# LewisClifton/Deep-Super-Resolution

Hardware: AMD Instinct MI355X
Metric: HR Mpixels/sec x4 GAN train step; PSNR delta vs reference (higher is better)
Workload: dtype bf16; 1 GPU; gan_x4: full GAN step x4 (G + D + VGG19 perceptual), batch 32/GPU, 128x128->512x512; global_batch=32, parallelism=dp1

## Files before the change

### deep-super-resolution_amd/csrc/conv_wgrad_tile.hip

```cpp
#include "dsr_common.h"
#include "dsr_kernels.h"

__device__ __forceinline__ s16x4 tr_read(const unsigned char* p) {
  return __builtin_amdgcn_ds_read_tr16_b64_v4i16((__attribute__((address_space(3))) s16x4*)(p));
}
__device__ __forceinline__ U4 tr_frag(const unsigned char* base, int p1, int p2, int chunk, int within) {
  s16x4 lo = tr_read(base + p1 * 128 + ((chunk ^ (p1 & 7)) << 4) + within);
  s16x4 hi = tr_read(base + p2 * 128 + ((chunk ^ (p2 & 7)) << 4) + within);
  return __builtin_bit_cast(U4, __builtin_shufflevector(lo, hi, 0, 1, 2, 3, 4, 5, 6, 7));
}

template <int DT, int KH, int KW, int S>
__global__ __launch_bounds__(256, 2) void conv_wgrad_tile_kernel(const WgradTileArgs a) {
  constexpr int R = (S == 1) ? 4 : 2;
  constexpr int HR = (R - 1) * S + KH, HC = 31 * S + KW;
  constexpr int NT = KH * KW;
  __shared__ __attribute__((aligned(16))) unsigned char sX[HR * HC * 128];
  __shared__ __attribute__((aligned(16))) unsigned char sY[R * 32 * 128];

  const int tid = threadIdx.x, lane = tid & 63, wave = __builtin_amdgcn_readfirstlane(tid >> 6);
  const int wr = wave >> 1, wc = wave & 1;
  const int g = lane >> 4, l16 = lane & 15, q4 = l16 >> 2, cc = 4 * (l16 & 3);
  const int pair = blockIdx.x;
  const int co0 = (pair / a.tiles_ci) * 64, ci0 = (pair % a.tiles_ci) * 64;
  const unsigned short* __restrict__ X = reinterpret_cast<const unsigned short*>(a.x);
  const unsigned short* __restrict__ DY = reinterpret_cast<const unsigned short*>(a.dy);

  f32x4 acc[NT][2][2];
#pragma unroll
  for (int t = 0; t < NT; ++t)
#pragma unroll
    for (int i = 0; i < 2; ++i)
#pragma unroll
      for (int j = 0; j < 2; ++j) acc[t][i][j] = f32x4{0.f, 0.f, 0.f, 0.f};

  const int c = tid & 7, pbase = tid >> 3;
  const bool yc_ok = (co0 + c * 8) < a.CoutP, xc_ok = (ci0 + c * 8) < a.CinP;
  int t_end = (blockIdx.y + 1) * a.tiles_per_block;
  if (t_end > a.ntiles) t_end = a.ntiles;
  const int per_img = a.tiles_y * a.tiles_x;

  for (int t = blockIdx.y * a.tiles_per_block; t < t_end; ++t) {
    const int n = t / per_img;
    const int rem = t - n * per_img;
    const int oy0 = (rem / a.tiles_x) * R, ox0 = (rem % a.tiles_x) * 32;
    __syncthreads();
#pragma unroll
    for (int i = 0; i < R * 32 * 8 / 256; ++i) {
      const int p = pbase + 32 * i;
      const int oy = oy0 + (p >> 5), ox = ox0 + (p & 31);
      const bool ok = yc_ok && oy < a.OH && ox < a.OW;
      U4 v = load16_or_zero(DY, ((size_t)(n * a.OH + oy) * a.OW + ox) * a.CoutP + co0 + c * 8, ok);
      *reinterpret_cast<U4*>(sY + p * 128 + ((c ^ (p & 7)) << 4)) = v;
    }
    {
      constexpr int NV = (HR * HC + 31) / 32;
      U4 v[NV];
#pragma unroll
      for (int u = 0; u < NV; ++u) {
        const int q = pbase + 32 * u;
        const int hr = q / HC, hc = q - hr * HC;
        bool ok = xc_ok && q < HR * HC;
        const int iy = pad_index(oy0 * S + hr - a.pad, a.IH, a.pad_mode, ok);
        const int ix = pad_index(ox0 * S + hc - a.pad, a.IW, a.pad_mode, ok);
        v[u] = load16_or_zero(X, ((size_t)(n * a.IH + iy) * a.IW + ix) * a.CinP + ci0 + c * 8, ok);
      }
#pragma unroll
      for (int u = 0; u < NV; ++u) {
        const int q = pbase + 32 * u;
        if (q < HR * HC) *reinterpret_cast<U4*>(sX + q * 128 + ((c ^ (q & 7)) << 4)) = v[u];
      }
    }
    __syncthreads();
#pragma unroll 1
    for (int r = 0; r < R; ++r) {
      U4 fa[2];
#pragma unroll
      for (int i = 0; i < 2; ++i) {
        const int ch = wr * 32 + i * 16 + cc;
        fa[i] = tr_frag(sY, r * 32 + 4 * g + q4, r * 32 + 16 + 4 * g + q4, ch >> 3, (ch & 7) * 2);
      }
#pragma unroll
      for (int kh = 0; kh < KH; ++kh)
#pragma unroll
        for (int kw = 0; kw < KW; ++kw) {
          const int qb = (r * S + kh) * HC + kw;
          const int q1 = qb + (4 * g + q4) * S, q2 = qb + (16 + 4 * g + q4) * S;
          U4 fb[2];
#pragma unroll
          for (int j = 0; j < 2; ++j) {
            const int ch = wc * 32 + j * 16 + cc;
            fb[j] = tr_frag(sX, q1, q2, ch >> 3, (ch & 7) * 2);
          }
#pragma unroll
          for (int i = 0; i < 2; ++i)
#pragma unroll
            for (int j = 0; j < 2; ++j) acc[kh * KW + kw][i][j] = mfma16<DT>(fa[i], fb[j], acc[kh * KW + kw][i][j]);
        }
    }
  }

  float* P = a.partial + (size_t)blockIdx.y * NT * a.CoutP * a.CinP;
#pragma unroll
  for (int t = 0; t < NT; ++t)
#pragma unroll
    for (int i = 0; i < 2; ++i)
#pragma unroll
      for (int j = 0; j < 2; ++j)
#pragma unroll
        for (int r = 0; r < 4; ++r) {
          const int co = co0 + wr * 32 + i * 16 + 4 * g + r, ci = ci0 + wc * 32 + j * 16 + l16;
          if (co < a.CoutP && ci < a.CinP) P[((size_t)t * a.CoutP + co) * a.CinP + ci] = acc[t][i][j][r];
        }
}

template <int DT>
__device__ __forceinline__ void conv_wgrad_dma_body(const WgradTileArgs& a, const int pair, const int ychunk) {
  constexpr int R = 2, HC = 40, HR = R + 2;
  constexpr int XB = HR * HC * 128, YB = R * 32 * 128, STAGE = XB + YB;
  __shared__ __attribute__((aligned(16))) unsigned char smem[2 * STAGE];

  const int tid = threadIdx.x, lane = tid & 63, wave = __builtin_amdgcn_readfirstlane(tid >> 6);
  const int g = lane >> 4, l16 = lane & 15, q4 = l16 >> 2, cc = 4 * (l16 & 3);
  const int co0 = (pair / a.tiles_ci) * 64, ci0 = (pair % a.tiles_ci) * 64;

  f32x4 acc[9][4];
#pragma unroll
  for (int t = 0; t < 9; ++t)
#pragma unroll
    for (int i = 0; i < 4; ++i) acc[t][i] = f32x4{0.f, 0.f, 0.f, 0.f};

  const int lp = 4 * g + q4;
  int offA[4], offB[3];
#pragma unroll
  for (int i = 0; i < 4; ++i) {
    const int ch = i * 16 + cc;
    offA[i] = XB + lp * 128 + (((ch >> 3) ^ (lp & 7)) << 4) + (ch & 7) * 2;
  }
#pragma unroll
  for (int kw = 0; kw < 3; ++kw) {
    const int ch = wave * 16 + cc;
    offB[kw] = lp * 128 + (((ch >> 3) ^ ((kw + lp) & 7)) << 4) + (ch & 7) * 2;
  }

  const int chunk = (tid & 7) ^ ((tid >> 3) & 7), pb = tid >> 3;
  const bool yc_ok = (co0 + chunk * 8) < a.CoutP, xc_ok = (ci0 + chunk * 8) < a.CinP;
  const BufSrd xrsrc = make_srd(const_cast<void*>(a.x), a.x_bytes);
  const BufSrd yrsrc = make_srd(const_cast<void*>(a.dy), a.dy_bytes);
  constexpr unsigned OOB = 0xFFFFFFF0u;
  typedef __attribute__((address_space(3))) void* lds_ptr;
  const int per_img = a.tiles_y * a.tiles_x;
  constexpr int NX = (HR * HC) / 32, NY = (R * 32) / 32;
  constexpr int FAR = 0x7FFFFF00;
  int xpart[NX], ypart[NY];
  unsigned hc_pack = 0;
#pragma unroll
  for (int u = 0; u < NX; ++u) {
    const int q = pb + 32 * u;
    const int hr = q / HC, hc = q - hr * HC;
    xpart[u] = (xc_ok && hc < 34) ? ((hr * a.IW + hc) * a.CinP + ci0 + chunk * 8) * 2 : FAR;
    hc_pack |= (unsigned)hc << (6 * u);
  }
#pragma unroll
  for (int u = 0; u < NY; ++u) {
    const int p = pb + 32 * u;
    ypart[u] = yc_ok ? (((p >> 5) * a.OW + (p & 31)) * a.CoutP + co0 + chunk * 8) * 2 : FAR;
  }
  const unsigned ximg = (unsigned)(a.IH * a.IW * a.CinP * 2), yimg = (unsigned)(a.OH * a.OW * a.CoutP * 2);
  const bool fast = a.pad_mode == DSR_PAD_ZERO;
  struct TileXY {
    int n, ty, tx;
  };
  auto dma = [&](const TileXY& tc, int buf) {
    const int n = tc.n;
    const int oy0 = tc.ty * R, ox0 = tc.tx * 32;
    unsigned char* st = smem + buf * STAGE;
    if (fast) {
      const BufSrd xr = make_srd(const_cast<unsigned char*>(reinterpret_cast<const unsigned char*>(a.x)) + (size_t)n * ximg, ximg);
      const BufSrd yr = make_srd(const_cast<unsigned char*>(reinterpret_cast<const unsigned char*>(a.dy)) + (size_t)n * yimg, yimg);
      const int xs = ((oy0 - a.pad) * a.IW + ox0 - a.pad) * a.CinP * 2;
      const int ys = (oy0 * a.OW + ox0) * a.CoutP * 2;
      unsigned char* dx = st + 8 * wave * 128;
      if (ox0 - a.pad >= 0 && ox0 - a.pad + 34 <= a.IW) {
#pragma unroll
        for (int u = 0; u < NX; ++u)
          lds_dma16(xr, dx + 32 * u * 128, (unsigned)(xpart[u] + xs));
      } else {
#pragma unroll
        for (int u = 0; u < NX; ++u) {
          const int ix = ox0 - a.pad + (int)((hc_pack >> (6 * u)) & 63);
          lds_dma16(xr, dx + 32 * u * 128, (unsigned)ix < (unsigned)a.IW ? (unsigned)(xpart[u] + xs) : OOB);
        }
      }
      if (ox0 + 32 <= a.OW) {
#pragma unroll
        for (int u = 0; u < NY; ++u)
          lds_dma16(yr, dx + XB + 32 * u * 128, (unsigned)(ypart[u] + ys));
      } else {
#pragma unroll
        for (int u = 0; u < NY; ++u)
          lds_dma16(yr, dx + XB + 32 * u * 128, ox0 + (pb & 31) < a.OW ? (unsigned)(ypart[u] + ys) : OOB);
      }
      return;
    }
#pragma unroll
    for (int u = 0; u < (HR * HC) / 32; ++u) {
      const int q = pb + 32 * u;
      const int hr = q / HC, hc = q - hr * HC;
      bool ok = xc_ok && hc < 34;
      const int iy = pad_index(oy0 + hr - a.pad, a.IH, a.pad_mode, ok);
      const int ix = pad_index(ox0 + hc - a.pad, a.IW, a.pad_mode, ok);
      lds_dma16(xrsrc, st + (32 * u + 8 * wave) * 128, ok ? (unsigned)((((n * a.IH + iy) * a.IW + ix) * a.CinP + ci0 + chunk * 8) * 2) : OOB);
    }
#pragma unroll
    for (int u = 0; u < (R * 32) / 32; ++u) {
      const int p = pb + 32 * u;
      const int oy = oy0 + (p >> 5), ox = ox0 + (p & 31);
      const bool ok = yc_ok && oy < a.OH && ox < a.OW;
      lds_dma16(yrsrc, st + XB + (32 * u + 8 * wave) * 128, ok ? (unsigned)((((n * a.OH + oy) * a.OW + ox) * a.CoutP + co0 + chunk * 8) * 2) : OOB);
    }
  };
  auto next_tile = [&](TileXY c) {
    if (++c.tx == a.tiles_x) {
      c.tx = 0;
      if (++c.ty == a.tiles_y) {
        c.ty = 0;
        ++c.n;
      }
    }
    return c;
  };

  int t = ychunk * a.tiles_per_block;
  int t_end = t + a.tiles_per_block;
  if (t_end > a.ntiles) t_end = a.ntiles;
  TileXY nxt;
  nxt.n = t / per_img;
  nxt.ty = (t - nxt.n * per_img) / a.tiles_x;
  nxt.tx = t - nxt.n * per_img - nxt.ty * a.tiles_x;
  __builtin_amdgcn_s_setprio(1);
  if (t < t_end) dma(nxt, 0);
  int buf = 0;
  for (; t < t_end; ++t, buf ^= 1) {
    asm volatile("s_waitcnt vmcnt(0)" ::: "memory");
    __builtin_amdgcn_s_barrier();
    asm volatile("" ::: "memory");
    nxt = next_tile(nxt);
    if (t + 1 < t_end) dma(nxt, buf ^ 1);
    __builtin_amdgcn_s_setprio(0);
    const unsigned char* st = smem + buf * STAGE;
    auto frag = [&](int off) {
      const s16x4 lo = tr_read(st + off);
      const s16x4 hi = tr_read(st + off + 2048);
      return __builtin_bit_cast(U4, __builtin_shufflevector(lo, hi, 0, 1, 2, 3, 4, 5, 6, 7));
    };
    constexpr int NU = 3 * HR;
    auto load_b = [&](int u) {
      const int kw = u / HR, h = u - kw * HR;
      return frag(offB[kw] + (h * HC + kw) * 128);
    };
    U4 fa[R][4], fb[3];
#pragma unroll
    for (int i = 0; i < 4; ++i) fa[0][i] = frag(offA[i]);
    fb[0] = load_b(0);
    fb[1] = load_b(1);
#pragma unroll
    for (int r = 1; r < R; ++r)
#pragma unroll
      for (int i = 0; i < 4; ++i) fa[r][i] = frag(offA[i] + r * 32 * 128);
#pragma unroll
    for (int u = 0; u < NU; ++u) {
      if (u + 2 < NU) fb[(u + 2) % 3] = load_b(u + 2);
      __builtin_amdgcn_sched_barrier(0);
      const int kw = u / HR, h = u - kw * HR;
#pragma unroll
      for (int r = 0; r < R; ++r) {
        const int kh = h - r;
        if (kh < 0 || kh > 2) continue;
#pragma unroll
        for (int i = 0; i < 4; ++i) acc[kh * 3 + kw][i] = mfma16<DT>(fa[r][i], fb[u % 3], acc[kh * 3 + kw][i]);
      }
      __builtin_amdgcn_sched_barrier(0);
    }
    __builtin_amdgcn_s_setprio(1);
  }

  float* P = a.partial + (size_t)ychunk * 9 * a.CoutP * a.CinP;
#pragma unroll
  for (int tp = 0; tp < 9; ++tp)
#pragma unroll
    for (int i = 0; i < 4; ++i)
#pragma unroll
      for (int r = 0; r < 4; ++r) {
        const int co = co0 + i * 16 + 4 * g + r, ci = ci0 + wave * 16 + l16;
        if (co < a.CoutP && ci < a.CinP) P[((size_t)tp * a.CoutP + co) * a.CinP + ci] = acc[tp][i][r];
      }
}

template <int DT>
__global__ __launch_bounds__(256, 2) void conv_wgrad_dma_kernel(const WgradTileArgs a) {
  conv_wgrad_dma_body<DT>(a, blockIdx.x, blockIdx.y);
}

template <int DT>
__global__ __launch_bounds__(256, 2) void conv_wgrad_dma_batch_kernel(const WgradBatchArgs b) {
  int pi = 0;
  while (pi + 1 < b.count && (int)blockIdx.x >= b.first_block[pi + 1]) ++pi;
  pi = __builtin_amdgcn_readfirstlane(pi);
  const WgradTileArgs a = b.p[pi];
  const int local = (int)blockIdx.x - b.first_block[pi];
  const int pairs = a.tiles_co * a.tiles_ci;
  conv_wgrad_dma_body<DT>(a, local % pairs, local / pairs);
}

template <int DT, int COH = 1>
__global__ __launch_bounds__(256 * COH, 2) void conv_wgrad_dma_s2_kernel(const WgradTileArgs a) {
  constexpr int HC = 80, HR = 3, NSLOT = HR * HC;
  constexpr int XB = NSLOT * 128, YB = 32 * 128, STAGE = XB + COH * YB;
  __shared__ __attribute__((aligned(16))) unsigned char smem[2 * STAGE];

  const int tid = threadIdx.x & 255, lane = tid & 63, wave = __builtin_amdgcn_readfirstlane((threadIdx.x >> 6) & 3);
  const int hsel = __builtin_amdgcn_readfirstlane(threadIdx.x >> 8);
  const int g = lane >> 4, l16 = lane & 15, q4 = l16 >> 2, cc = 4 * (l16 & 3);
  const int pair = blockIdx.x;
  const int co0 = (pair / a.tiles_ci) * 64 * COH + hsel * 64, ci0 = (pair % a.tiles_ci) * 64;

  f32x4 acc[9][4];
#pragma unroll
  for (int t = 0; t < 9; ++t)
#pragma unroll
    for (int i = 0; i < 4; ++i) acc[t][i] = f32x4{0.f, 0.f, 0.f, 0.f};

  const int lp = 4 * g + q4;
  int offA[4], offB[2];
#pragma unroll
  for (int i = 0; i < 4; ++i) {
    const int ch = i * 16 + cc;
    offA[i] = XB + hsel * YB + lp * 128 + (((ch >> 3) ^ (lp & 7)) << 4) + (ch & 7) * 2;
  }
#pragma unroll
  for (int v = 0; v < 2; ++v) {
    const int ch = wave * 16 + cc;
    offB[v] = 2 * lp * 128 + (((ch >> 3) ^ ((lp + v) & 7)) << 4) + (ch & 7) * 2;
  }

  const int pb = tid >> 3;
  const int xchunk = (tid & 7) ^ ((4 * wave + (lane >> 4)) & 7);
  const int ychunk = (tid & 7) ^ ((tid >> 3) & 7);
  const bool yc_ok = (co0 + ychunk * 8) < a.CoutP, xc_ok = (ci0 + xchunk * 8) < a.CinP;
  const BufSrd xrsrc = make_srd(const_cast<void*>(a.x), a.x_bytes);
  const BufSrd yrsrc = make_srd(const_cast<void*>(a.dy), a.dy_bytes);
  constexpr unsigned OOB = 0xFFFFFFF0u;
  typedef __attribute__((address_space(3))) void* lds_ptr;
  const int per_img = a.tiles_y * a.tiles_x;
  constexpr int NX = (NSLOT + 31) / 32;
  constexpr int FAR = 0x7FFFFF00;
  int xpart[NX];
  unsigned hc_lo = 0, hc_hi = 0;
#pragma unroll
  for (int u = 0; u < NX; ++u) {
    const int q = pb + 32 * u;
    const int hr = q / HC, hc = q - hr * HC;
    xpart[u] = (xc_ok && hc < 65 && hr < HR) ? ((hr * a.IW + hc) * a.CinP + ci0 + xchunk * 8) * 2 : FAR;
    if (u < 4) hc_lo |= (unsigned)hc << (7 * u);
    else hc_hi |= (unsigned)hc << (7 * (u - 4));
  }
  const int ypart = yc_ok ? (pb * a.CoutP + co0 + ychunk * 8) * 2 : FAR;
  const unsigned ximg = (unsigned)(a.IH * a.IW * a.CinP * 2), yimg = (unsigned)(a.OH * a.OW * a.CoutP * 2);
  const bool fast = a.pad_mode == DSR_PAD_ZERO;
  struct TileXY {
    int n, ty, tx;
  };
  auto dma = [&](const TileXY& tc, int buf) {
    const int n = tc.n, oy0 = tc.ty, ox0 = tc.tx * 32;
    unsigned char* st = smem + buf * STAGE;
    if (fast) {
      const BufSrd xr = make_srd(const_cast<unsigned char*>(reinterpret_cast<const unsigned char*>(a.x)) + (size_t)n * ximg, ximg);
      const BufSrd yr = make_srd(const_cast<unsigned char*>(reinterpret_cast<const unsigned char*>(a.dy)) + (size_t)n * yimg, yimg);
      const int ix0 = ox0 * 2 - a.pad;
      const int xs = ((oy0 * 2 - a.pad) * a.IW + ix0) * a.CinP * 2;
      const int ys = (oy0 * a.OW + ox0) * a.CoutP * 2;
      unsigned char* dx = st + 8 * wave * 128;
      const bool interior = ix0 >= 0 && ix0 + 65 <= a.IW;
#pragma unroll
      for (int u = 0; u < NX; ++u) {
        if (COH == 2 && (u & 1) != hsel) continue;
        if (32 * u + 8 * wave < NSLOT) {
          unsigned off = (unsigned)(xpart[u] + xs);
          if (!interior) {
            const int hc = (int)(((u < 4 ? hc_lo >> (7 * u) : hc_hi >> (7 * (u - 4)))) & 127);
            if (!((unsigned)(ix0 + hc) < (unsigned)a.IW)) off = OOB;
          }
          lds_dma16(xr, dx + 32 * u * 128, off);
        }
      }
      lds_dma16(yr, dx + XB + hsel * YB, (ox0 + 32 <= a.OW || ox0 + pb < a.OW) ? (unsigned)(ypart + ys) : OOB);
      return;
    }
#pragma unroll
    for (int u = 0; u < (NSLOT + 31) / 32; ++u) {
      if (COH == 2 && (u & 1) != hsel) continue;
      if (32 * u + 8 * wave < NSLOT) {
        const int q = pb + 32 * u;
        const int hr = q / HC, hc = q - hr * HC;
        bool ok = xc_ok && hc < 65;
        const int iy = pad_index(oy0 * 2 + hr - a.pad, a.IH, a.pad_mode, ok);
        const int ix = pad_index(ox0 * 2 + hc - a.pad, a.IW, a.pad_mode, ok);
        lds_dma16(xrsrc, st + (32 * u + 8 * wave) * 128, ok ? (unsigned)((((n * a.IH + iy) * a.IW + ix) * a.CinP + ci0 + xchunk * 8) * 2) : OOB);
      }
    }
    {
      const int ox = ox0 + pb;
      const bool ok = yc_ok && ox < a.OW;
      lds_dma16(yrsrc, st + XB + hsel * YB + 8 * wave * 128, ok ? (unsigned)((((n * a.OH + oy0) * a.OW + ox) * a.CoutP + co0 + ychunk * 8) * 2) : OOB);
    }
  };

  int t = blockIdx.y * a.tiles_per_block;
  int t_end = t + a.tiles_per_block;
  if (t_end > a.ntiles) t_end = a.ntiles;
  TileXY nxt;
  nxt.n = t / per_img;
  nxt.ty = (t - nxt.n * per_img) / a.tiles_x;
  nxt.tx = t - nxt.n * per_img - nxt.ty * a.tiles_x;
  __builtin_amdgcn_s_setprio(1);
  if (t < t_end) dma(nxt, 0);
  int buf = 0;
  for (; t < t_end; ++t, buf ^= 1) {
    asm volatile("s_waitcnt vmcnt(0)" ::: "memory");
    __builtin_amdgcn_s_barrier();
    asm volatile("" ::: "memory");
    if (++nxt.tx == a.tiles_x) {
      nxt.tx = 0;
      if (++nxt.ty == a.tiles_y) {
        nxt.ty = 0;
        ++nxt.n;
      }
    }
    if (t + 1 < t_end) dma(nxt, buf ^ 1);
    __builtin_amdgcn_s_setprio(0);
    const unsigned char* st = smem + buf * STAGE;
    U4 fa[4], fb[3];
    auto load_b = [&](int u) {
      const int kh = u / 3, kw = u % 3;
      const s16x4 lo = tr_read(st + offB[kw >> 1] + (kh * HC + kw) * 128);
      const s16x4 hi = tr_read(st + offB[kw >> 1] + (kh * HC + kw) * 128 + 32 * 128);
      return __builtin_bit_cast(U4, __builtin_shufflevector(lo, hi, 0, 1, 2, 3, 4, 5, 6, 7));
    };
#pragma unroll
    for (int i = 0; i < 4; ++i) {
      const s16x4 lo = tr_read(st + offA[i]);
      const s16x4 hi = tr_read(st + offA[i] + 2048);
      fa[i] = __builtin_bit_cast(U4, __builtin_shufflevector(lo, hi, 0, 1, 2, 3, 4, 5, 6, 7));
    }
    fb[0] = load_b(0);
    fb[1] = load_b(1);
#pragma unroll
    for (int u = 0; u < 9; ++u) {
      if (u + 2 < 9) fb[(u + 2) % 3] = load_b(u + 2);
      __builtin_amdgcn_sched_barrier(0);
#pragma unroll
      for (int i = 0; i < 4; ++i) acc[u][i] = mfma16<DT>(fa[i], fb[u % 3], acc[u][i]);
      __builtin_amdgcn_sched_barrier(0);
    }
    __builtin_amdgcn_s_setprio(1);
  }

  float* P = a.partial + (size_t)blockIdx.y * 9 * a.CoutP * a.CinP;
#pragma unroll
  for (int tp = 0; tp < 9; ++tp)
#pragma unroll
    for (int i = 0; i < 4; ++i)
#pragma unroll
      for (int r = 0; r < 4; ++r) {
        const int co = co0 + i * 16 + 4 * g + r, ci = ci0 + wave * 16 + l16;
        if (co < a.CoutP && ci < a.CinP) P[((size_t)tp * a.CoutP + co) * a.CinP + ci] = acc[tp][i][r];
      }
}

static bool dsr_wgrad_s2_co128(int KH, int stride, int CoutP, long long x_bytes) {
  const char* e = getenv("DSR_WGRAD_S2_CO128");
  const int mode = e ? atoi(e) : 1;
  if (mode == 0 || KH != 3 || stride != 2 || CoutP < 128 || CoutP % 128 != 0) return false;
  return mode == 2 || x_bytes >= 400ll * 1000 * 1000;
}

int dsr_wgrad_tile_plan(int KH, int KW, int stride, int N, int OH, int OW, int CinP, int CoutP, WgradTileArgs* a) {
  const bool k3 = KH == 3 && KW == 3 && (stride == 1 || stride == 2);
  const bool k1 = KH == 1 && KW == 1 && stride == 1;
  if (!k3 && !k1) return 0;
  const int R = k1 ? 4 : (stride == 1 ? 2 : 1);
  a->tiles_y = (OH + R - 1) / R;
  a->tiles_x = (OW + 31) / 32;
  a->ntiles = N * a->tiles_y * a->tiles_x;
  const bool co128 = dsr_wgrad_s2_co128(KH, stride, CoutP, (long long)N * (2 * OH) * (2 * OW) * CinP * 2);
  a->tiles_co = co128 ? CoutP / 128 : (CoutP + 63) / 64;
  a->tiles_ci = (CinP + 63) / 64;
  long long pairs = (long long)a->tiles_co * a->tiles_ci;
  long long want = ((co128 ? 256 : 512) + pairs - 1) / pairs;
  if (want > a->ntiles) want = a->ntiles;
  if (want < 1) want = 1;
  a->tiles_per_block = (int)((a->ntiles + want - 1) / want);
  return (a->ntiles + a->tiles_per_block - 1) / a->tiles_per_block;
}

template <int DT>
static void launch_dt(const WgradTileArgs& a, int KH, int stride, dim3 grid, hipStream_t st) {
  if (KH == 3 && stride == 1)
    hipLaunchKernelGGL((conv_wgrad_dma_kernel<DT>), grid, dim3(256), 0, st, a);
  else if (KH == 3 && a.tiles_co * 128 == a.CoutP && a.tiles_co * 64 != a.CoutP)
    hipLaunchKernelGGL((conv_wgrad_dma_s2_kernel<DT, 2>), grid, dim3(512), 0, st, a);
  else if (KH == 3)
    hipLaunchKernelGGL((conv_wgrad_dma_s2_kernel<DT>), grid, dim3(256), 0, st, a);
  else
    hipLaunchKernelGGL((conv_wgrad_tile_kernel<DT, 1, 1, 1>), grid, dim3(256), 0, st, a);
}

void dsr_launch_wgrad_dma_batch(const WgradBatchArgs& b, int dtype, hipStream_t st) {
  const int blocks = b.first_block[b.count];
  if (dtype == DSR_DTYPE_BF16)
    hipLaunchKernelGGL((conv_wgrad_dma_batch_kernel<DSR_DTYPE_BF16>), dim3(blocks), dim3(256), 0, st, b);
  else
    hipLaunchKernelGGL((conv_wgrad_dma_batch_kernel<DSR_DTYPE_F16>), dim3(blocks), dim3(256), 0, st, b);
}

void dsr_launch_wgrad_tile(const WgradTileArgs& a, int KH, int stride, int ychunks, int dtype, hipStream_t st) {
  dim3 grid(a.tiles_co * a.tiles_ci, ychunks);
  if (dtype == DSR_DTYPE_BF16)
    launch_dt<DSR_DTYPE_BF16>(a, KH, stride, grid, st);
  else
    launch_dt<DSR_DTYPE_F16>(a, KH, stride, grid, st);
}
```

### deep-super-resolution_amd/csrc/dsr_kernels.h

```cpp
#pragma once
#include <hip/hip_runtime.h>
#include <stdint.h>
#include <stdlib.h>

#define DSR_MAX_TAPS 96
#define DSR_WGRAD_SCRATCH_SLABS 16

#define DSR_F_BIAS 1
#define DSR_F_STATS 2
#define DSR_F_PIXSHUF 4
#define DSR_F_OUT_NCHW_F32 8
#define DSR_F_PRELU_PTR 16
#define DSR_F_AFFINE 32
#define DSR_F_RESIDUAL 64
#define DSR_F_MASK 128

struct FastDiv {
  unsigned magic;
  unsigned shift;
};
static inline FastDiv fd_make(unsigned d) {
  FastDiv f;
  unsigned s = 0;
  while ((1ull << s) < d) ++s;
  f.shift = s;
  f.magic = (unsigned)((((1ull << 32) * ((1ull << s) - d)) / d) + 1);
  return f;
}
#if defined(__HIPCC__)
__device__ __forceinline__ int fd_div(const FastDiv f, int m) {
  return (int)((__umulhi((unsigned)m, f.magic) + (unsigned)m) >> f.shift);
}
#endif

struct ConvGemmArgs {
  const void* x;
  const void* w;
  void* y;
  float* out_f32;
  const float* bias;
  const float* prelu;
  float* stats;
  unsigned x_bytes, w_bytes;
  unsigned y_bytes;
  int M, GH, GW;
  int IH, IW, CinP;
  int OH, OW, CoutP;
  int NB;
  int cout;
  int stats_stride;
  int isy, isx, osy, osx, ooy, oox;
  int ntaps, CU, U, ksteps;
  int pad_mode, act;
  float slope;
  int flags;
  int tiles_m, tiles_n;
  FastDiv fd_ghw, fd_gw, fd_cu, fd_cu8;
  const void* mask_x;
  int mask_act;
  float mask_slope;
  int taps[DSR_MAX_TAPS];
};

void dsr_launch_conv_gemm(const ConvGemmArgs& a, int dtype, hipStream_t st);
static inline int dsr_conv_big_mode(void) {
  const char* e = getenv("DSR_CONV_BIG");
  return e ? atoi(e) : 2;
}
static inline bool dsr_conv_gemm_use_256(long long M, int NB, bool fast, bool stats) {
  const long long tiles = ((M + 255) / 256) * ((NB + 255) / 256);
  (void)stats;
  const char* t = getenv("DSR_CONV_BIG_TILES");
  return dsr_conv_big_mode() == 2 && fast && NB % 256 == 0 && tiles >= (t ? atoi(t) : 150);
}

static inline bool dsr_conv_gemm_use_224(long long M, int NB, bool fast, int flags) {
  const char* e = getenv("DSR_CONV_BM224");
  const int mode = e ? atoi(e) : 1;
  if (mode == 0 || (flags & (DSR_F_STATS | DSR_F_PIXSHUF | DSR_F_OUT_NCHW_F32))) return false;
  if (!dsr_conv_gemm_use_256(M, NB, fast, false)) return false;
  if (mode == 2) return true;
  const long long cus = 256, nt = NB / 256;
  const long long r256 = (((M + 255) / 256) * nt + cus - 1) / cus, r224 = (((M + 223) / 224) * nt + cus - 1) / cus;
  return r224 * 7 < r256 * 8;
}

static inline bool dsr_conv_gemm_use_64(long long M, int NB, bool fast, int flags) {
  const char* e = getenv("DSR_CONV_BM64");
  const int mode = e ? atoi(e) : 1;
  if (mode == 0 || !fast || NB % 128 != 0 || (flags & (DSR_F_STATS | DSR_F_PIXSHUF | DSR_F_OUT_NCHW_F32))) return false;
  if (mode == 2) return true;
  return ((M + 127) / 128) * (NB / 128) < 256;
}

bool dsr_launch_conv_gemm_persist(const ConvGemmArgs& a, int dtype, hipStream_t st);

struct WgradArgs {
  const void* x;
  const void* dy;
  float* partial;
  int M, OH, OW, IH, IW, CinP, CoutP;
  int stride, pad, pad_mode, KH, KW;
  int tiles_co, tiles_ci, splits, chunk;
  FastDiv fd_ohw, fd_ow;
};
void dsr_launch_wgrad(const WgradArgs& a, int dtype, hipStream_t st);

struct WgradTileArgs {
  const void* x;
  const void* dy;
  float* partial;
  int N, OH, OW, IH, IW, CinP, CoutP;
  int pad, pad_mode;
  int tiles_co, tiles_ci;
  int tiles_y, tiles_x, ntiles, tiles_per_block;
  unsigned x_bytes, dy_bytes;
};
#define DSR_WGRAD_BATCH_MAX 36
struct WgradBatchArgs {
  WgradTileArgs p[DSR_WGRAD_BATCH_MAX];
  int first_block[DSR_WGRAD_BATCH_MAX + 1];
  int count;
};
static_assert(sizeof(WgradBatchArgs) <= 4096, "kernel arguments are limited to 4 KB");
void dsr_launch_wgrad_dma_batch(const WgradBatchArgs& b, int dtype, hipStream_t st);
struct WgradReduceBatchArgs {
  struct Entry {
    const float* partial;
    float* dw;
    int splits, Cout, Cin, CoutP, CinP, first_block;
  } e[DSR_WGRAD_BATCH_MAX];
  int count, total_blocks;
};
void dsr_launch_wgrad_reduce_batch(const WgradReduceBatchArgs& r, hipStream_t st);
int dsr_wgrad_tile_plan(int KH, int KW, int stride, int N, int OH, int OW, int CinP, int CoutP, WgradTileArgs* a);
void dsr_launch_wgrad_tile(const WgradTileArgs& a, int KH, int stride, int ychunks, int dtype, hipStream_t st);

int dsr_wgrad_toeplitz_plan(int N, int H, int W, WgradTileArgs* a);
void dsr_launch_wgrad_toeplitz(const WgradTileArgs& a, int dtype, hipStream_t st);
void dsr_launch_dgrad_toeplitz(const void* dy, const void* w_dgrad, void* dx, int N, int H, int W, int dtype, hipStream_t st,
                               const void* act_out = nullptr, const float* prelu = nullptr, void* dyu = nullptr,
                               float* ps_partial = nullptr);
int dsr_dgrad_toeplitz_ps_blocks(int N, int H, int W);
int dsr_wgrad_taps_plan(int KH, int KW, int stride, int N, int OH, int OW, int CinP, int CoutP, WgradTileArgs* a);
void dsr_launch_wgrad_taps(const WgradTileArgs& a, int KH, int ychunks, int dtype, hipStream_t st);

struct SmallNArgs {
  const void* x;
  const void* w;
  void* y;
  float* out_f32;
  const float* bias;
  const float* prelu;
  int IH, IW, CinP, OH, OW, CoutP, NB, cout, KH, KW, pad, act;
  float slope;
  int tiles_y, tiles_x, ntiles;
  int flip;
  unsigned x_bytes;
};
int dsr_launch_conv_smalln(SmallNArgs& a, int N, int dtype, hipStream_t st);

struct C64Args {
  const void* x;
  const void* w;
  void* y;
  const float* bias;
  const float* prelu;
  float* stats;
  const float* scale;
  const float* shift;
  const void* res;
  int H, W;
  int CoutP;
  int act;
  float slope;
  int flags;
  int mask_act;
  float mask_slope;
  int tiles_y, tiles_x, ntiles;
  int tap_y[9], tap_x[9];
  unsigned x_bytes, y_bytes;
};
int dsr_c64_tiles(int N, int H, int W, int tile_rows);
int dsr_c64_stat_rows(int N, int H, int W, int CoutP);
void dsr_launch_conv_c64(C64Args& a, int N, int dtype, hipStream_t st);

struct Cin8Args {
  const void* x;
  const void* w;
  void* y;
  const float* bias;
  const float* prelu;
  int H, W;
  int act;
  float slope;
  int tiles_y, tiles_x, ntiles;
  unsigned x_bytes;
  int nt_store;
};
void dsr_launch_conv_cin8(Cin8Args& a, int N, int dtype, hipStream_t st);
int dsr_conv_rgb9_supported(int KH, int KW, int stride, int pad, int pad_mode, int Cin, int Cout);
void dsr_launch_conv_rgb9(Cin8Args& a, int N, int dtype, hipStream_t st);
struct Rgb9WgradArgs {
  const void* x;
  const void* dy;
  float* partial;
  int H, W;
  int tiles_y, tiles_x, ntiles;
  unsigned x_bytes, dy_bytes;
};
int dsr_wgrad_rgb9_blocks(int N, int H, int W);
size_t dsr_wgrad_rgb9_slab_floats();
void dsr_launch_wgrad_rgb9(Rgb9WgradArgs& a, int N, int Cin, float* dw, int dtype, hipStream_t st);

struct DgradS2Args {
  const void* dy;
  const void* w;
  void* dx;
  int H, W, CinP, CoutP;
  int OH, OW, M, ci_blocks, kblocks, tiles_m;
  unsigned dy_bytes, w_bytes, dx_bytes;
  FastDiv fd_ghw, fd_gw;
  const void* img;
  const float* w0;
  const float* b0;
  float* fb_partial;
  unsigned img_bytes;
  int Cin0, act0;
  float slope0;
  const void* bn_y;
  const float* bn_scale;
  const float* bn_shift;
  float* bn_partial;
  int bn_act;
  float bn_slope;
};
int dsr_dgrad_s2_blocks(int N, int H, int W, int CinP);
bool dsr_dgrad_s2_bn_supported(int KH, int KW, int stride, int pad, int pad_mode, int H, int W, int CinP, int CoutP, int N);
bool dsr_dgrad_s2_supported(int KH, int KW, int stride, int pad, int pad_mode, int H, int W, int CinP, int CoutP, int N);
void dsr_launch_dgrad_s2(DgradS2Args& a, int N, int dtype, hipStream_t st);

struct Halo64Args {
  const void* x;
  const void* w;
  void* y;
  const float* bias;
  int H, W, CinP;
  int mirror;
  int act;
  float slope;
  int flags;
  const void* mask_x;
  int mask_act;
  float mask_slope;
  int cout_full;
  int kblocks, tiles_y, tiles_x, ntiles;
  unsigned w_bytes, y_bytes;
};
bool dsr_halo64_supported(int KH, int KW, int stride, int pad, int pad_mode, int H, int W, int CinP, int CoutP);
void dsr_launch_conv_halo64(Halo64Args& a, int N, int dtype, hipStream_t st);

struct First2Args {
  const void* x;
  const void* w0;
  const float* b0;
  float slope0;
  const void* w1;
  const float* b1;
  void* a0;
  void* y1;
  float* stats;
  int H, W, OH, OW, tiles_y, tiles_x, ntiles;
  unsigned a0_bytes, y1_bytes;
};

struct FirstBwdArgs {
  const void* x;
  const void* dout;
  const void* y;
  float* partial;
  int N, H, W, act;
  float slope;
  int tiles_y, tiles_x, ntiles;
  unsigned x_bytes, y_bytes;
  const float* w0;
  const float* b0;
  int Cin;
};

void dsr_launch_wgrad_reduce(const float* partial, float* dw, int splits, int ntaps, int Cout, int Cin, int CoutP,
                             int CinP, hipStream_t st);

#include <atomic>
struct LdsOptIn {
  std::atomic<unsigned long long> done{0};
  void ensure(const void* fn, int bytes) {
    int dev = 0;
    (void)hipGetDevice(&dev);
    const unsigned long long bit = 1ull << (dev & 63);
    if (!(done.load(std::memory_order_acquire) & bit)) {
      (void)hipFuncSetAttribute(fn, hipFuncAttributeMaxDynamicSharedMemorySize, bytes);
      done.fetch_or(bit, std::memory_order_release);
    }
  }
};

int dsr_launch_status(const char* what);
int dsr_fail(int code, const char* fmt, ...);

#define DSR_REQUIRE(cond, ...)                          \
  do {                                                  \
    if (!(cond)) return dsr_fail(DSR_E_ARG, __VA_ARGS__); \
  } while (0)
#define DSR_DTYPE_OK(dt) ((dt) == DSR_DTYPE_BF16 || (dt) == DSR_DTYPE_F16)
#define DSR_CP_OK(Cp) ((Cp) >= 8 && (Cp) % 8 == 0 && (Cp) <= 2048)
```

Baseline: 247.3 HR Mpixels/s.

## Process two output rows per stride-2 wgrad tile to reuse shared input halo

The stride-2 3x3 weight-gradient kernel now tiles two output rows at a time. The 5-row input halo is loaded once and shared between both rows instead of loading 3 rows per output row, which cuts global-to-LDS traffic. The block index is remapped so consecutive tiles stay on the same XCD, and co128 is forced on in two-row mode. The non-co128 two-row variant splits its rows across two 256-thread halves that write separate partial slabs, which doubles the partial buffer and the reduction work. It also raises register pressure from the larger fa array.

```diff
diff --git a/deep-super-resolution_amd/csrc/conv_wgrad_tile.hip b/deep-super-resolution_amd/csrc/conv_wgrad_tile.hip
--- a/deep-super-resolution_amd/csrc/conv_wgrad_tile.hip
+++ b/deep-super-resolution_amd/csrc/conv_wgrad_tile.hip
@@ -313,17 +313,29 @@
   conv_wgrad_dma_body<DT>(a, local % pairs, local / pairs);
 }
 
-template <int DT, int COH = 1>
-__global__ __launch_bounds__(256 * COH, 2) void conv_wgrad_dma_s2_kernel(const WgradTileArgs a) {
-  constexpr int HC = 80, HR = 3, NSLOT = HR * HC;
-  constexpr int XB = NSLOT * 128, YB = 32 * 128, STAGE = XB + COH * YB;
+template <int DT, int COH, int R>
+__global__ __launch_bounds__((COH == 2 || R == 2) ? 512 : 256, 2) void conv_wgrad_dma_s2_kernel(const WgradTileArgs a) {
+  constexpr int HALVES = (COH == 2 || R == 2) ? 2 : 1;
+  constexpr int RW = COH == 2 ? R : 1;
+  constexpr int HC = 80, HR = 2 * R + 1, NSLOT = HR * HC;
+  constexpr int YB = 32 * 128;
+  constexpr int XB = NSLOT * 128, STAGE = XB + COH * R * YB;
   __shared__ __attribute__((aligned(16))) unsigned char smem[2 * STAGE];
 
   const int tid = threadIdx.x & 255, lane = tid & 63, wave = __builtin_amdgcn_readfirstlane((threadIdx.x >> 6) & 3);
   const int hsel = __builtin_amdgcn_readfirstlane(threadIdx.x >> 8);
+  const int coh = COH == 2 ? hsel : 0;
+  const int row0 = COH == 2 ? 0 : hsel;
   const int g = lane >> 4, l16 = lane & 15, q4 = l16 >> 2, cc = 4 * (l16 & 3);
-  const int pair = blockIdx.x;
-  const int co0 = (pair / a.tiles_ci) * 64 * COH + hsel * 64, ci0 = (pair % a.tiles_ci) * 64;
+  int pair, chunk;
+  {
+    const int total = gridDim.x * gridDim.y, hw = blockIdx.x + blockIdx.y * gridDim.x;
+    const int q = total >> 3, rem = total & 7, xcd = hw & 7, slot = hw >> 3;
+    const int lin = xcd < rem ? xcd * (q + 1) + slot : rem * (q + 1) + (xcd - rem) * q + slot;
+    pair = __builtin_amdgcn_readfirstlane(lin % (int)gridDim.x);
+    chunk = __builtin_amdgcn_readfirstlane(lin / (int)gridDim.x);
+  }
+  const int co0 = (pair / a.tiles_ci) * 64 * COH + coh * 64, ci0 = (pair % a.tiles_ci) * 64;
 
   f32x4 acc[9][4];
 #pragma unroll
@@ -336,12 +348,12 @@
 #pragma unroll
   for (int i = 0; i < 4; ++i) {
     const int ch = i * 16 + cc;
-    offA[i] = XB + hsel * YB + lp * 128 + (((ch >> 3) ^ (lp & 7)) << 4) + (ch & 7) * 2;
+    offA[i] = XB + (coh * R + row0) * YB + lp * 128 + (((ch >> 3) ^ (lp & 7)) << 4) + (ch & 7) * 2;
   }
 #pragma unroll
   for (int v = 0; v < 2; ++v) {
     const int ch = wave * 16 + cc;
-    offB[v] = 2 * lp * 128 + (((ch >> 3) ^ ((lp + v) & 7)) << 4) + (ch & 7) * 2;
+    offB[v] = (2 * row0 * HC + 2 * lp) * 128 + (((ch >> 3) ^ ((lp + v) & 7)) << 4) + (ch & 7) * 2;
   }
 
   const int pb = tid >> 3;
@@ -351,28 +363,32 @@
   const BufSrd xrsrc = make_srd(const_cast<void*>(a.x), a.x_bytes);
   const BufSrd yrsrc = make_srd(const_cast<void*>(a.dy), a.dy_bytes);
   constexpr unsigned OOB = 0xFFFFFFF0u;
-  typedef __attribute__((address_space(3))) void* lds_ptr;
   const int per_img = a.tiles_y * a.tiles_x;
   constexpr int NX = (NSLOT + 31) / 32;
+  constexpr int NXL = HALVES == 2 ? (NX + 1) / 2 : NX;
+  static_assert(NXL <= 8, "halo column packing holds 8 passes");
   constexpr int FAR = 0x7FFFFF00;
-  int xpart[NX];
+  int xpart[NXL];
   unsigned hc_lo = 0, hc_hi = 0;
 #pragma unroll
-  for (int u = 0; u < NX; ++u) {
+  for (int k = 0; k < NXL; ++k) {
+    const int u = HALVES == 2 ? 2 * k + hsel : k;
     const int q = pb + 32 * u;
     const int hr = q / HC, hc = q - hr * HC;
-    xpart[u] = (xc_ok && hc < 65 && hr < HR) ? ((hr * a.IW + hc) * a.CinP + ci0 + xchunk * 8) * 2 : FAR;
-    if (u < 4) hc_lo |= (unsigned)hc << (7 * u);
-    else hc_hi |= (unsigned)hc << (7 * (u - 4));
+    xpart[k] = (xc_ok && hc < 65 && hr < HR) ? ((hr * a.IW + hc) * a.CinP + ci0 + xchunk * 8) * 2 : FAR;
+    if (k < 4) hc_lo |= (unsigned)hc << (7 * k);
+    else hc_hi |= (unsigned)hc << (7 * (k - 4));
   }
   const int ypart = yc_ok ? (pb * a.CoutP + co0 + ychunk * 8) * 2 : FAR;
   const unsigned ximg = (unsigned)(a.IH * a.IW * a.CinP * 2), yimg = (unsigned)(a.OH * a.OW * a.CoutP * 2);
+  const int yrow = a.OW * a.CoutP * 2;
   const bool fast = a.pad_mode == DSR_PAD_ZERO;
   struct TileXY {
     int n, ty, tx;
   };
+  auto fetches_row = [&](int r) { return COH == 2 || R == 1 || r == hsel; };
   auto dma = [&](const TileXY& tc, int buf) {
-    const int n = tc.n, oy0 = tc.ty, ox0 = tc.tx * 32;
+    const int n = tc.n, oy0 = tc.ty * R, ox0 = tc.tx * 32;
     unsigned char* st = smem + buf * STAGE;
     if (fast) {
       const BufSrd xr = make_srd(const_cast<unsigned char*>(reinterpret_cast<const unsigned char*>(a.x)) + (size_t)n * ximg, ximg);
@@ -383,23 +399,26 @@
       unsigned char* dx = st + 8 * wave * 128;
       const bool interior = ix0 >= 0 && ix0 + 65 <= a.IW;
 #pragma unroll
-      for (int u = 0; u < NX; ++u) {
-        if (COH == 2 && (u & 1) != hsel) continue;
+      for (int k = 0; k < NXL; ++k) {
+        const int u = HALVES == 2 ? 2 * k + hsel : k;
         if (32 * u + 8 * wave < NSLOT) {
-          unsigned off = (unsigned)(xpart[u] + xs);
+          unsigned off = (unsigned)(xpart[k] + xs);
           if (!interior) {
-            const int hc = (int)(((u < 4 ? hc_lo >> (7 * u) : hc_hi >> (7 * (u - 4)))) & 127);
+            const int hc = (int)(((k < 4 ? hc_lo >> (7 * k) : hc_hi >> (7 * (k - 4)))) & 127);
             if (!((unsigned)(ix0 + hc) < (unsigned)a.IW)) off = OOB;
           }
           lds_dma16(xr, dx + 32 * u * 128, off);
         }
       }
-      lds_dma16(yr, dx + XB + hsel * YB, (ox0 + 32 <= a.OW || ox0 + pb < a.OW) ? (unsigned)(ypart + ys) : OOB);
+      const bool col_ok = ox0 + 32 <= a.OW || ox0 + pb < a.OW;
+#pragma unroll
+      for (int r = 0; r < R; ++r)
+        if (fetches_row(r)) lds_dma16(yr, dx + XB + (coh * R + r) * YB, col_ok ? (unsigned)(ypart + ys + r * yrow) : OOB);
       return;
     }
 #pragma unroll
-    for (int u = 0; u < (NSLOT + 31) / 32; ++u) {
-      if (COH == 2 && (u & 1) != hsel) continue;
+    for (int k = 0; k < NXL; ++k) {
+      const int u = HALVES == 2 ? 2 * k + hsel : k;
       if (32 * u + 8 * wave < NSLOT) {
         const int q = pb + 32 * u;
         const int hr = q / HC, hc = q - hr * HC;
@@ -409,14 +428,17 @@
         lds_dma16(xrsrc, st + (32 * u + 8 * wave) * 128, ok ? (unsigned)((((n * a.IH + iy) * a.IW + ix) * a.CinP + ci0 + xchunk * 8) * 2) : OOB);
       }
     }
-    {
-      const int ox = ox0 + pb;
-      const bool ok = yc_ok && ox < a.OW;
-      lds_dma16(yrsrc, st + XB + hsel * YB + 8 * wave * 128, ok ? (unsigned)((((n * a.OH + oy0) * a.OW + ox) * a.CoutP + co0 + ychunk * 8) * 2) : OOB);
-    }
+#pragma unroll
+    for (int r = 0; r < R; ++r)
+      if (fetches_row(r)) {
+        const int oy = oy0 + r, ox = ox0 + pb;
+        const bool ok = yc_ok && oy < a.OH && ox < a.OW;
+        lds_dma16(yrsrc, st + XB + (coh * R + r) * YB + 8 * wave * 128,
+                  ok ? (unsigned)((((n * a.OH + oy) * a.OW + ox) * a.CoutP + co0 + ychunk * 8) * 2) : OOB);
+      }
   };
 
-  int t = blockIdx.y * a.tiles_per_block;
+  int t = chunk * a.tiles_per_block;
   int t_end = t + a.tiles_per_block;
   if (t_end > a.ntiles) t_end = a.ntiles;
   TileXY nxt;
@@ -440,33 +462,43 @@
     if (t + 1 < t_end) dma(nxt, buf ^ 1);
     __builtin_amdgcn_s_setprio(0);
     const unsigned char* st = smem + buf * STAGE;
-    U4 fa[4], fb[3];
+    constexpr int HRW = 2 * RW + 1, NU = 3 * HRW;
+    U4 fa[RW][4], fb[3];
     auto load_b = [&](int u) {
-      const int kh = u / 3, kw = u % 3;
-      const s16x4 lo = tr_read(st + offB[kw >> 1] + (kh * HC + kw) * 128);
-      const s16x4 hi = tr_read(st + offB[kw >> 1] + (kh * HC + kw) * 128 + 32 * 128);
+      const int kw = u / HRW, h = u - kw * HRW;
+      const s16x4 lo = tr_read(st + offB[kw >> 1] + (h * HC + kw) * 128);
+      const s16x4 hi = tr_read(st + offB[kw >> 1] + (h * HC + kw) * 128 + 32 * 128);
       return __builtin_bit_cast(U4, __builtin_shufflevector(lo, hi, 0, 1, 2, 3, 4, 5, 6, 7));
     };
 #pragma unroll
-    for (int i = 0; i < 4; ++i) {
-      const s16x4 lo = tr_read(st + offA[i]);
-      const s16x4 hi = tr_read(st + offA[i] + 2048);
-      fa[i] = __builtin_bit_cast(U4, __builtin_shufflevector(lo, hi, 0, 1, 2, 3, 4, 5, 6, 7));
-    }
+    for (int r = 0; r < RW; ++r)
+#pragma unroll
+      for (int i = 0; i < 4; ++i) {
+        const s16x4 lo = tr_read(st + offA[i] + r * YB);
+        const s16x4 hi = tr_read(st + offA[i] + r * YB + 2048);
+        fa[r][i] = __builtin_bit_cast(U4, __builtin_shufflevector(lo, hi, 0, 1, 2, 3, 4, 5, 6, 7));
+      }
     fb[0] = load_b(0);
     fb[1] = load_b(1);
 #pragma unroll
-    for (int u = 0; u < 9; ++u) {
-      if (u + 2 < 9) fb[(u + 2) % 3] = load_b(u + 2);
+    for (int u = 0; u < NU; ++u) {
+      if (u + 2 < NU) fb[(u + 2) % 3] = load_b(u + 2);
       __builtin_amdgcn_sched_barrier(0);
-#pragma unroll
-      for (int i = 0; i < 4; ++i) acc[u][i] = mfma16<DT>(fa[i], fb[u % 3], acc[u][i]);
+      const int kw = u / HRW, h = u - kw * HRW;
+#pragma unroll
+      for (int r = 0; r < RW; ++r) {
+        const int kh = h - 2 * r;
+        if (kh < 0 || kh > 2) continue;
+#pragma unroll
+        for (int i = 0; i < 4; ++i) acc[kh * 3 + kw][i] = mfma16<DT>(fa[r][i], fb[u % 3], acc[kh * 3 + kw][i]);
+      }
       __builtin_amdgcn_sched_barrier(0);
     }
     __builtin_amdgcn_s_setprio(1);
   }
 
-  float* P = a.partial + (size_t)blockIdx.y * 9 * a.CoutP * a.CinP;
+  constexpr int SPLIT = (COH == 1 && R == 2) ? 2 : 1;
+  float* P = a.partial + (size_t)(chunk * SPLIT + (SPLIT == 2 ? hsel : 0)) * 9 * a.CoutP * a.CinP;
 #pragma unroll
   for (int tp = 0; tp < 9; ++tp)
 #pragma unroll
@@ -478,40 +510,54 @@
       }
 }
 
-static bool dsr_wgrad_s2_co128(int KH, int stride, int CoutP, long long x_bytes) {
+static int dsr_wgrad_s2_rows() {
+  const char* e = getenv("DSR_WGRAD_S2_ROWS");
+  return (e && atoi(e) == 1) ? 1 : 2;
+}
+
+static bool dsr_wgrad_s2_co128(int KH, int stride, int CoutP, long long x_bytes, int rows) {
   const char* e = getenv("DSR_WGRAD_S2_CO128");
   const int mode = e ? atoi(e) : 1;
   if (mode == 0 || KH != 3 || stride != 2 || CoutP < 128 || CoutP % 128 != 0) return false;
-  return mode == 2 || x_bytes >= 400ll * 1000 * 1000;
+  return mode == 2 || rows == 2 || x_bytes >= 400ll * 1000 * 1000;
 }
 
 int dsr_wgrad_tile_plan(int KH, int KW, int stride, int N, int OH, int OW, int CinP, int CoutP, WgradTileArgs* a) {
   const bool k3 = KH == 3 && KW == 3 && (stride == 1 || stride == 2);
   const bool k1 = KH == 1 && KW == 1 && stride == 1;
   if (!k3 && !k1) return 0;
-  const int R = k1 ? 4 : (stride == 1 ? 2 : 1);
+  const int R = k1 ? 4 : (stride == 1 ? 2 : dsr_wgrad_s2_rows());
+  a->s2_rows = (k3 && stride == 2) ? R : 0;
   a->tiles_y = (OH + R - 1) / R;
   a->tiles_x = (OW + 31) / 32;
   a->ntiles = N * a->tiles_y * a->tiles_x;
-  const bool co128 = dsr_wgrad_s2_co128(KH, stride, CoutP, (long long)N * (2 * OH) * (2 * OW) * CinP * 2);
+  const bool co128 = dsr_wgrad_s2_co128(KH, stride, CoutP, (long long)N * (2 * OH) * (2 * OW) * CinP * 2, a->s2_rows);
   a->tiles_co = co128 ? CoutP / 128 : (CoutP + 63) / 64;
   a->tiles_ci = (CinP + 63) / 64;
   long long pairs = (long long)a->tiles_co * a->tiles_ci;
-  long long want = ((co128 ? 256 : 512) + pairs - 1) / pairs;
+  const bool wide = co128 || a->s2_rows == 2;
+  long long want = ((wide ? 256 : 512) + pairs - 1) / pairs;
   if (want > a->ntiles) want = a->ntiles;
   if (want < 1) want = 1;
   a->tiles_per_block = (int)((a->ntiles + want - 1) / want);
-  return (a->ntiles + a->tiles_per_block - 1) / a->tiles_per_block;
+  const int blocks_y = (a->ntiles + a->tiles_per_block - 1) / a->tiles_per_block;
+  return (a->s2_rows == 2 && !co128) ? 2 * blocks_y : blocks_y;
 }
 
 template <int DT>
-static void launch_dt(const WgradTileArgs& a, int KH, int stride, dim3 grid, hipStream_t st) {
+static void launch_dt(const WgradTileArgs& a, int KH, int stride, int ychunks, hipStream_t st) {
+  dim3 grid(a.tiles_co * a.tiles_ci, ychunks);
+  const bool co128 = a.tiles_co * 128 == a.CoutP && a.tiles_co * 64 != a.CoutP;
   if (KH == 3 && stride == 1)
     hipLaunchKernelGGL((conv_wgrad_dma_kernel<DT>), grid, dim3(256), 0, st, a);
-  else if (KH == 3 && a.tiles_co * 128 == a.CoutP && a.tiles_co * 64 != a.CoutP)
-    hipLaunchKernelGGL((conv_wgrad_dma_s2_kernel<DT, 2>), grid, dim3(512), 0, st, a);
+  else if (KH == 3 && a.s2_rows == 2 && co128)
+    hipLaunchKernelGGL((conv_wgrad_dma_s2_kernel<DT, 2, 2>), grid, dim3(512), 0, st, a);
+  else if (KH == 3 && a.s2_rows == 2)
+    hipLaunchKernelGGL((conv_wgrad_dma_s2_kernel<DT, 1, 2>), dim3(grid.x, ychunks / 2), dim3(512), 0, st, a);
+  else if (KH == 3 && co128)
+    hipLaunchKernelGGL((conv_wgrad_dma_s2_kernel<DT, 2, 1>), grid, dim3(512), 0, st, a);
   else if (KH == 3)
-    hipLaunchKernelGGL((conv_wgrad_dma_s2_kernel<DT>), grid, dim3(256), 0, st, a);
+    hipLaunchKernelGGL((conv_wgrad_dma_s2_kernel<DT, 1, 1>), grid, dim3(256), 0, st, a);
   else
     hipLaunchKernelGGL((conv_wgrad_tile_kernel<DT, 1, 1, 1>), grid, dim3(256), 0, st, a);
 }
@@ -525,9 +571,8 @@
 }
 
 void dsr_launch_wgrad_tile(const WgradTileArgs& a, int KH, int stride, int ychunks, int dtype, hipStream_t st) {
-  dim3 grid(a.tiles_co * a.tiles_ci, ychunks);
   if (dtype == DSR_DTYPE_BF16)
-    launch_dt<DSR_DTYPE_BF16>(a, KH, stride, grid, st);
+    launch_dt<DSR_DTYPE_BF16>(a, KH, stride, ychunks, st);
   else
-    launch_dt<DSR_DTYPE_F16>(a, KH, stride, grid, st);
-}
+    launch_dt<DSR_DTYPE_F16>(a, KH, stride, ychunks, st);
+}
diff --git a/deep-super-resolution_amd/csrc/dsr_kernels.h b/deep-super-resolution_amd/csrc/dsr_kernels.h
--- a/deep-super-resolution_amd/csrc/dsr_kernels.h
+++ b/deep-super-resolution_amd/csrc/dsr_kernels.h
@@ -115,6 +115,7 @@
   int tiles_co, tiles_ci;
   int tiles_y, tiles_x, ntiles, tiles_per_block;
   unsigned x_bytes, dy_bytes;
+  int s2_rows;
 };
 #define DSR_WGRAD_BATCH_MAX 36
 struct WgradBatchArgs {
```

Result: no change. 249.3 HR Mpixels/s, median of 6 (+0.8%).
